# Leo-Liao-Chao/Uncertainty-Aware-CILQR-for-Trajectory-Optimization

Hardware: AMD Instinct MI355X
Metric: CILQR solves/sec (N=50, batch B) (higher is better)
Workload: dtype f64

## Files before the change

### uncertainty-aware-cilqr-for-trajectory-optimization_amd/csrc/cilqr_solve.hip

```cpp
#include <type_traits>

#include "cilqr_device.hpp"

namespace cilqr {

using namespace dev;

namespace {

constexpr int FREC = 16;

__device__ __forceinline__ double readfirstlane_f64(double v) {
  int lo = __double2loint(v), hi = __double2hiint(v);
  lo = __builtin_amdgcn_readfirstlane(lo);
  hi = __builtin_amdgcn_readfirstlane(hi);
  return __hiloint2double(hi, lo);
}

__device__ __forceinline__ double wave_sum(double v) {
#pragma unroll
  for (int o = 32; o > 0; o >>= 1) v += __shfl_xor(v, o, WAVE);
  return v;
}

// ... 358 lines not shown
    riccati_step<!GENERAL>(rb, V, dt, two_wvel, lamb, g, ok);
    if (GENERAL) { if (!ok) return false; } else suspect |= __builtin_amdgcn_ballot_w64(!ok);
    store_gains<RW>(kK, j - 1, g);
  }
  if (j == 0) {
    riccati_step<!GENERAL>(ra, V, dt, two_wvel, lamb, g, ok);
    if (GENERAL) { if (!ok) return false; } else suspect |= __builtin_amdgcn_ballot_w64(!ok);
    store_gains<RW>(kK, 0, g);
  }
  return suspect == 0;
}

#define CILQR_MFMA(xa, xb, xc) __builtin_amdgcn_mfma_f64_4x4x4f64(xa, xb, xc, 0, 0, 0)

__device__ __forceinline__ double readlane_f64(double v, int l) {
  int lo = __double2loint(v), hi = __double2hiint(v);
  lo = __builtin_amdgcn_readlane(lo, l);
  hi = __builtin_amdgcn_readlane(hi, l);
  return __hiloint2double(hi, lo);
}
__device__ __forceinline__ double odd_blocks_from_even(double v) {
  int lo = __double2loint(v), hi = __double2hiint(v);
  lo = __builtin_amdgcn_update_dpp(lo, lo, 0x114, 0xF, 0xA, false);
  hi = __builtin_amdgcn_update_dpp(hi, hi, 0x114, 0xF, 0xA, false);
  return __hiloint2double(hi, lo);
}

struct MfmaOperands { double AB, AA, BB, Ca, Cb; };
struct MfmaCursor {
  const double *AB, *AA, *BB, *Ca, *Cb;
  int sAB, sAA, sBB, sCa, sCb;
  __device__ __forceinline__ void upper(MfmaOperands& o) const { o.AB = AB[RECF]; o.AA = AA[RECF]; o.BB = BB[RECF]; o.Ca = Ca[RECF]; o.Cb = Cb[RECF]; }
  __device__ __forceinline__ void lower(MfmaOperands& o) const { o.AB = AB[0]; o.AA = AA[0]; o.BB = BB[0]; o.Ca = Ca[0]; o.Cb = Cb[0]; }
  __device__ __forceinline__ void back() { AB -= sAB; AA -= sAA; BB -= sBB; Ca -= sCa; Cb -= sCb; }
};

__device__ __forceinline__ void mfma_place(const double*& ptr, int& stride, int slot, const double* low, const double* cst) {
  ptr = slot >= 0 ? low + slot : cst + (-1 - slot);
  stride = slot >= 0 ? 2 * RECF : 0;
}

template <bool FSMEM, bool DIAG>
__device__ __forceinline__ bool riccati_mfma(int N, const double* rec, double* kK, double* fwd, const double* cst, double inv_half_dt, double lamb_in,
                                             unsigned long long* sub) {
  constexpr int C0 = -1, C1 = -2, CDT = -3, CW = -4, C2 = -5;
  const int lane = threadIdx.x;
  const int e = ((lane >> 4) << 2) | (lane & 3);
  const bool odd = (lane & 4) != 0;
  const int slotA = e == 0 || e == 5 || e == 10 || e == 15 ? C1 : e == 2 ? 10 : e == 6 ? 11 : e == 3 ? 12 : e == 7 ? 13 : C0;
  const int slotB = e == 0 ? 10 : e == 4 ? 11 : e == 8 ? C2 : e == 13 ? CDT : C0;
  const int slotXX = e == 0 ? 3 : e == 1 || e == 4 ? 4 : e == 5 ? 5 : e == 10 ? CW : C0;
  const int slotX = e == 2 ? 0 : e == 6 ? 1 : e == 10 ? 2 : C0;
  const int slotUU = e == 0 ? 8 : e == 5 ? 9 : e == 2 ? 6 : e == 6 ? 7 : C0;
  const double* low = rec + (N - 2) * RECF;
  MfmaCursor cur;
  mfma_place(cur.AB, cur.sAB, odd ? slotB : slotA, low, cst);
  mfma_place(cur.AA, cur.sAA, slotA, low, cst);
  mfma_place(cur.BB, cur.sBB, slotB, low, cst);
  mfma_place(cur.Ca, cur.sCa, odd ? slotX : slotXX, low, cst);
  mfma_place(cur.Cb, cur.sCb, odd ? slotUU : C0, low, cst);
  double m00 = e == 0 ? 1.0 : 0.0, m01 = e == 1 || e == 4 ? 1.0 : 0.0, m11 = e == 5 ? 1.0 : 0.0;
  double mvc = odd && (lane & 3) == 2 ? 1.0 : 0.0;
  double lamb = lamb_in, lamb0 = lamb_in * (inv_half_dt * inv_half_dt);
  double lamb_row = (lane >> 4) == 0 ? lamb0 : lamb;
  CILQR_PIN(m00); CILQR_PIN(m01); CILQR_PIN(m11); CILQR_PIN(mvc); CILQR_PIN(lamb); CILQR_PIN(lamb0); CILQR_PIN(lamb_row);
  const bool stores = lane == 6 || lane == 22 || lane < 4 || (lane >= 16 && lane < 20);
  const int gslot = lane == 6 ? 0 : lane == 22 ? 1 : lane < 4 ? 2 + lane : 6 + (lane & 3);
  unsigned goff = stores ? (unsigned)(((N - 1) * FREC + gslot) * 8) : (unsigned)((N * FREC + (lane & 15)) * 8);
  const unsigned gstride = stores ? FREC * 8 : 0;
  char* const gbase = reinterpret_cast<char*>(fwd);
  double* gp = kK + (N - 1) * RECF + (stores ? gslot : 10 + (lane & 3));

  MfmaOperands oa, ob;
  cur.upper(oa);
  double V = odd_blocks_from_even(oa.Ca), vc = oa.Ca * mvc;
  int signs_v = 0, signs_s = 0;
  double det0 = 0.0;
  auto step = [&](const MfmaOperands& o) {
    unsigned long long s0 = 0, s1 = 0, s2 = 0, s3 = 0;
    if (DIAG) stamp_request(s0, V);
    const double P = CILQR_MFMA(V, o.AB, vc);
    const double Db = CILQR_MFMA(o.BB, P, o.Cb);
    const double Da = CILQR_MFMA(o.AA, P, o.Ca);
    const double a = readlane_f64(Db, 4), b = readlane_f64(Db, 5), d = readlane_f64(Db, 21);
    if (DIAG) stamp_request(s1, a + b + d);
    const double bb = b * b;
    det0 = fma(a, d, -bb);
    signs_v |= __double2hiint(det0);
    signs_s |= __double2hiint(a) | __double2hiint(d);
    const double ar = a + lamb0, dr = d + lamb;
    const double nr = -rcp_newton(fma(ar, dr, -bb));
    if (DIAG) stamp_request(s2, nr);
    const double adj = fma(ar, m11, fma(-b, m01, dr * m00));
    const double Dk = CILQR_MFMA(adj, Db, 0.0) * nr;
    const double H0 = fma(lamb_row, Dk, Db);
    const double H = odd_blocks_from_even(H0);
    double Dv = CILQR_MFMA(H, Dk, Da);
    vc = Dv * mvc;
    CILQR_PIN(vc);
    CILQR_PIN(Dv);
    V = odd_blocks_from_even(Dv);
    if (FSMEM) {
      *reinterpret_cast<double*>(gbase + goff) = Dk;
      goff -= gstride;
      asm volatile("" : "+v"(goff));
    } else {
      *gp = Dk;
      gp -= RECF;
    }
    if (DIAG) {
      stamp_request(s3, V);
      stamps_collect(s0, s1, s2, s3);
      sub[5] += s1 - s0; sub[6] += s2 - s1; sub[7] += s3 - s2;
    }
  };
  auto trip = [&] {
    cur.lower(ob);
    step(oa);
    cur.back();
    cur.upper(oa);
    step(ob);
  };
  bool two_left;
  if (FSMEM) {
    two_left = ((N - 1) & 1) != 0;
    for (int trips = (N - 1) >> 1; trips > 0; --trips) trip();
  } else {
    int j = N - 1;
    for (; j >= 2; j -= 2) trip();
    two_left = j == 1;
  }
  if (two_left) {
    cur.lower(ob);
    step(oa);
    step(ob);
  } else {
    step(oa);
  }
  return __builtin_amdgcn_ballot_w64((signs_v | signs_s) < 0 || !(det0 == det0)) == 0;
}

typedef __attribute__((address_space(3))) double lds_f64;
struct MfmaLdsCursor {
  const lds_f64 *AB, *AA, *BB, *Ca, *Cb;
  int sAB, sAA, sBB, sCa, sCb;
  __device__ __forceinline__ void upper(MfmaOperands& o) const { o.AB = AB[RECF]; o.AA = AA[RECF]; o.BB = BB[RECF]; o.Ca = Ca[RECF]; o.Cb = Cb[RECF]; }
  __device__ __forceinline__ void lower(MfmaOperands& o) const { o.AB = AB[0]; o.AA = AA[0]; o.BB = BB[0]; o.Ca = Ca[0]; o.Cb = Cb[0]; }
};
__device__ __forceinline__ void mfma_place(const lds_f64*& ptr, int& stride, int slot, const lds_f64* low, const lds_f64* cst) {
  ptr = slot >= 0 ? low + slot : cst + (-1 - slot);
  stride = slot >= 0 ? 2 * RECF : 0;
}

template <bool DIAG>
__device__ __forceinline__ bool riccati_mfma_smem(int N, const double* rec, double* fwd, const double* cst, double inv_half_dt, double lamb_in,
                                                  unsigned long long* sub) {
  constexpr int C0 = -1, C1 = -2, CDT = -3, CW = -4, C2 = -5;
  const int lane = threadIdx.x;
  const int e = ((lane >> 4) << 2) | (lane & 3);
  const bool odd = (lane & 4) != 0;
  const int slotA = e == 0 || e == 5 || e == 10 || e == 15 ? C1 : e == 2 ? 10 : e == 6 ? 11 : e == 3 ? 12 : e == 7 ? 13 : C0;
  const int slotB = e == 0 ? 10 : e == 4 ? 11 : e == 8 ? C2 : e == 13 ? CDT : C0;
  const int slotXX = e == 0 ? 3 : e == 1 || e == 4 ? 4 : e == 5 ? 5 : e == 10 ? CW : C0;
  const int slotX = e == 2 ? 0 : e == 6 ? 1 : e == 10 ? 2 : C0;
  const int slotUU = e == 0 ? 8 : e == 5 ? 9 : e == 2 ? 6 : e == 6 ? 7 : C0;
  using PTR = const lds_f64*;
  const PTR low = (PTR)rec + (N - 2) * RECF;
  const PTR cstp = (PTR)cst;
  MfmaLdsCursor cur;
  mfma_place(cur.AB, cur.sAB, odd ? slotB : slotA, low, cstp);
  mfma_place(cur.AA, cur.sAA, slotA, low, cstp);
  mfma_place(cur.BB, cur.sBB, slotB, low, cstp);
  mfma_place(cur.Ca, cur.sCa, odd ? slotX : slotXX, low, cstp);
  mfma_place(cur.Cb, cur.sCb, odd ? slotUU : C0, low, cstp);
  double m00 = e == 0 ? 1.0 : 0.0, m01 = e == 1 || e == 4 ? 1.0 : 0.0, m11 = e == 5 ? 1.0 : 0.0;
  double mvc = odd && (lane & 3) == 2 ? 1.0 : 0.0;
  double lamb = lamb_in, lamb0 = lamb_in * (inv_half_dt * inv_half_dt);
  double lamb_row = (lane >> 4) == 0 ? lamb0 : lamb;
  CILQR_PIN(m00); CILQR_PIN(m01); CILQR_PIN(m11); CILQR_PIN(mvc); CILQR_PIN(lamb); CILQR_PIN(lamb0); CILQR_PIN(lamb_row);
  const bool stores = lane == 6 || lane == 22 || lane < 4 || (lane >= 16 && lane < 20);
  const int gslot = lane == 6 ? 0 : lane == 22 ? 1 : lane < 4 ? 2 + lane : 6 + (lane & 3);
  unsigned goff = stores ? (unsigned)(((N - 1) * FREC + gslot) * 8) : (unsigned)((N * FREC + (lane & 15)) * 8);
  const unsigned gstride = stores ? FREC * 8 : 0;
  char* const gbase = reinterpret_cast<char*>(fwd);
  lds_f64* qp = (lds_f64*)rec + (N - 2) * RECF + (lane == 4 ? 0 : lane == 5 ? 1 : lane == 21 ? 2 : 3 + lane % 11);

  MfmaOperands oa, ob;
  cur.upper(oa);
  double V = odd_blocks_from_even(oa.Ca), vc = oa.Ca * mvc;
  auto step = [&](const MfmaOperands& o, auto kind, auto upper_step) {
    constexpr int KIND = decltype(kind)::value, QOFF = decltype(upper_step)::value ? RECF : 0;
    unsigned long long s0 = 0, s1 = 0, s2 = 0, s3 = 0;
    if (DIAG) stamp_request(s0, V);
    const double P = CILQR_MFMA(V, o.AB, vc);
    double Db = CILQR_MFMA(o.BB, P, o.Cb);
    const double Da = CILQR_MFMA(o.AA, P, o.Ca);
    if (KIND != 3) {
      asm volatile("" : "+v"(Db) : "v"(cur.AB), "v"(cur.AA), "v"(cur.BB), "v"(cur.Ca), "v"(cur.Cb));
      if (KIND == 1) cur.upper(oa); else cur.lower(ob);
      asm volatile("");
    }
    const double a = readlane_f64(Db, 4), b = readlane_f64(Db, 5), d = readlane_f64(Db, 21);
    if (DIAG) stamp_request(s1, a + b + d);
    const double bb = b * b;
    const double ar = a + lamb0, dr = d + lamb;
    const double den = fma(ar, dr, -bb);
    const double adj = fma(ar, m11, fma(-b, m01, dr * m00));
    double Dkr = CILQR_MFMA(adj, Db, 0.0);
    double r = __builtin_amdgcn_rcp(den);
    asm volatile("" : "+v"(Dkr), "+v"(r), "+v"(goff) : "v"(qp));
    qp[QOFF] = Db;
    asm volatile("");
    r = fma(fma(-den, r, 1.0), r, r);
    r = fma(fma(-den, r, 1.0), r, r);
    const double nr = -r;
    if (DIAG) stamp_request(s2, nr);
    const double Dk = Dkr * nr;
    double H0 = fma(lamb_row, Dk, Db);
    if (KIND == 0) {
      asm volatile("" : "+v"(H0) : "v"(cur.AB), "v"(cur.AA));
      cur.AB -= cur.sAB; cur.AA -= cur.sAA;
    }
    if (KIND == 1) {
      asm volatile("" : "+v"(H0) : "v"(qp));
      qp -= 2 * RECF;
    }
    double H = odd_blocks_from_even(H0);
    if (KIND == 0) {
      asm volatile("" : "+v"(H) : "v"(cur.BB), "v"(cur.Ca));
      cur.BB -= cur.sBB; cur.Ca -= cur.sCa;
    }
    double Dv = CILQR_MFMA(H, Dk, Da);
    asm volatile("" : "+v"(Dv) : "v"(goff));
    *reinterpret_cast<double*>(gbase + goff) = Dk;
    asm volatile("" : "+v"(Dv) : : "memory");
    vc = Dv * mvc;
    CILQR_PIN(vc);
    asm volatile("" : "+v"(Dv) : "v"(goff), "v"(cur.Cb));
    goff -= gstride;
    if (KIND == 0) cur.Cb -= cur.sCb;
    V = odd_blocks_from_even(Dv);
    if (DIAG) {
      stamp_request(s3, V);
      stamps_collect(s0, s1, s2, s3);
      sub[5] += s1 - s0; sub[6] += s2 - s1; sub[7] += s3 - s2;
    }
  };
  using Upper = std::true_type;
  using Lower = std::false_type;
  using K0 = std::integral_constant<int, 0>;
  using K1 = std::integral_constant<int, 1>;
  using K2 = std::integral_constant<int, 2>;
  using K3 = std::integral_constant<int, 3>;
  for (int trips = (N - 1) >> 1; trips > 0; --trips) {
    step(oa, K0(), Upper());
    step(ob, K1(), Lower());
  }
  if (((N - 1) & 1) != 0) {
    step(oa, K2(), Upper());
    step(ob, K3(), Lower());
  } else {
    step(oa, K3(), Upper());
  }
  bool bad = false;
  for (int base = 0; base < N; base += WAVE) {
    const int t = base + lane;
    const double* q = rec + (t < N ? t : N - 1) * RECF;
    const double a = q[0], b = q[1], d = q[2];
    const double bb = b * b;
    const double det0 = fma(a, d, -bb);
    const int signs = __double2hiint(det0) | __double2hiint(a) | __double2hiint(d);
    bad |= t < N && (signs < 0 || (t == 0 && !(det0 == det0)));
  }
  return __builtin_amdgcn_ballot_w64(bad) == 0;
}

template <int KS>
__device__ __forceinline__ void load_fwd(FwdIn& o, const double* X, const double* U, const double* kK, int i) {
  const double* xo = X + i * XR;
  o.x = xo[0]; o.y = xo[1]; o.v = xo[2]; o.th = xo[3];
  o.u0 = U[2 * i]; o.u1 = U[2 * i + 1];
  const double* g = kK + i * KS;
#pragma unroll
  for (int k = 0; k < KR; ++k) o.g[k] = g[k];
}

__device__ __forceinline__ void fwd_step_store(const FwdConst& k, const FwdIn& c, State& s, double& max_turn, double inv_half_dt,
                                               double* Un_i, double* Xn_next) {
  double u0, u1;
  forward_step<true>(k, c, s, max_turn, u0, u1, inv_half_dt);
  Un_i[0] = u0; Un_i[1] = u1;
  Xn_next[0] = s.x; Xn_next[1] = s.y; Xn_next[2] = s.v; Xn_next[3] = s.th; Xn_next[4] = s.c; Xn_next[5] = s.s;
}

typedef double d2_t __attribute__((ext_vector_type(2)));
typedef __attribute__((address_space(3))) d2_t lds_d2;
constexpr int FSTEP = FREC * 8;
static_assert(XR % 2 == 0, "state records are whole 16-byte pairs");
struct FwdBump {
  unsigned& off;
  lds_d2*& un;
  lds_d2*& xn;
  template <int J> __device__ __forceinline__ void pin(double& ps, double& pc) const {
    if (J == 0) {
      asm volatile("" : "+v"(ps), "+v"(pc) : "v"(un));
      un += 2;
      asm volatile("" : "+v"(un));
    } else if (J == 1) {
      asm volatile("" : "+v"(ps), "+v"(pc) : "v"(xn));
      xn += XR;
      asm volatile("" : "+v"(xn));
    } else if (J == 2) {
      asm volatile("" : "+v"(ps), "+v"(pc) : "s"(off));
      off += 2 * FSTEP;
      asm volatile("" : "+s"(off));
    } else {
      CILQR_PIN2(ps, pc);
    }
  }
};
typedef double d8_t __attribute__((ext_vector_type(8)));
struct FwdS { d8_t lo, hi; };
__device__ __forceinline__ void f_sload_first(FwdS& r, const double* p) {
  asm volatile("s_load_dwordx16 %0, %2, 0x0\n\ts_load_dwordx16 %1, %2, 0x40" : "=&s"(r.lo), "=&s"(r.hi) : "s"(p) : "memory");
}
template <int AHEAD>
__device__ __forceinline__ void f_sload_next(FwdS& r, const double* fwd, unsigned off) {
  asm volatile("s_load_dwordx16 %0, %2, %3 offset:%4\n\ts_load_dwordx16 %1, %2, %3 offset:%5"
               : "+s"(r.lo), "+s"(r.hi) : "s"(fwd), "s"(off), "n"(AHEAD), "n"(AHEAD + 64) : "memory");
}
__device__ __forceinline__ void f_swait(FwdS& r) {
  __builtin_amdgcn_s_waitcnt(0xC07F);
  asm volatile("" : "+s"(r.lo), "+s"(r.hi) : : "memory");
}
__device__ __forceinline__ void f_sunpack(FwdIn& o, const FwdS& r) {
  o.g[0] = r.lo[0]; o.g[1] = r.lo[1]; o.g[2] = r.lo[2]; o.g[3] = r.lo[3]; o.g[4] = r.lo[4]; o.g[5] = r.lo[5];
  o.g[6] = r.lo[6]; o.g[7] = r.lo[7]; o.g[8] = r.hi[0]; o.g[9] = r.hi[1];
  o.x = r.hi[2]; o.y = r.hi[3]; o.v = r.hi[4]; o.th = r.hi[5]; o.u0 = r.hi[6]; o.u1 = r.hi[7];
}

template <bool PUBLISH = false>
__device__ __forceinline__ bool forward_smem(const KParams& kp, int N, const double* X, const double* fwd, double* Xn, double* Un) {
  asm volatile("s_waitcnt vmcnt(0)\n\ts_dcache_inv\n\ts_waitcnt lgkmcnt(0)" ::: "memory");
  FwdConst k;
  make_fwd_const(k, kp);
  double ihd = 2.0 / kp.dt;
  CILQR_PIN(ihd);
  State s;
  s.x = X[0]; s.y = X[1]; s.v = X[2]; s.th = X[3]; s.c = X[4]; s.s = X[5];
  store_state(Xn, 0, s);
  double max_turn = 0.0;
  FwdS r;
  FwdIn c;
  f_sload_first(r, fwd);
  unsigned off = 0;
  lds_d2* un = (lds_d2*)Un;
  lds_d2* xn = (lds_d2*)(Xn + XR);
  asm volatile("" : "+s"(off), "+v"(un), "+v"(xn));
  const FwdBump bump{off, un, xn};
  auto step = [&](auto ahead, auto slot, const auto& pins) {
    constexpr int AHEAD = decltype(ahead)::value, SLOT = decltype(slot)::value;
    f_swait(r);
    f_sunpack(c, r);
    double u0, u1;
    forward_controls_scalar(c, s, u0, u1, ihd);
    f_sload_next<AHEAD>(r, fwd, off);
    un[SLOT] = d2_t{u0, u1};
    const double delta = dyn_pose_loop(k, s, u0, u1, max_turn);
    lds_d2* xo = xn + SLOT * (XR / 2);
    xo[0] = d2_t{s.x, s.y};
    if (PUBLISH) asm volatile("" ::: "memory");
    xo[1] = d2_t{s.v, s.th};
    rotate_heading(k, delta, s.s, s.c, pins);
    CILQR_PIN2(s.s, s.c);
  };
  using I0 = std::integral_constant<int, 0>;
  using I1 = std::integral_constant<int, 1>;
  const unsigned end = (unsigned)N * FSTEP, last = N > 0 ? end - FSTEP : 0;
  while (off < last) {
    step(std::integral_constant<int, FSTEP>(), I0(), PlainPins());
    step(std::integral_constant<int, 2 * FSTEP>(), I1(), bump);
  }
  if (off < end) step(std::integral_constant<int, FSTEP>(), I0(), PlainPins());
  f_swait(r);
  return max_turn <= MAX_TURN;
}

template <int KS>
__device__ __forceinline__ bool forward_fast(const KParams& kp, int N, const double* X, const double* U, const double* kK,
                                             double* Xn, double* Un) {
  FwdConst k;
  make_fwd_const(k, kp);
  double ihd = 2.0 / kp.dt;
  CILQR_PIN(ihd);
  State s;
  s.x = X[0]; s.y = X[1]; s.v = X[2]; s.th = X[3]; s.c = X[4]; s.s = X[5];
  if (threadIdx.x == 0) store_state(Xn, 0, s);
  double max_turn = 0.0;
  FwdIn fa, fb;
  load_fwd<KS>(fa, X, U, kK, 0);
  int i = 0;
  for (; i + 1 < N; i += 2) {
    load_fwd<KS>(fb, X, U, kK, i + 1);
    fwd_step_store(k, fa, s, max_turn, ihd, Un + 2 * i, Xn + (i + 1) * XR);
    load_fwd<KS>(fa, X, U, kK, i + 2 < N ? i + 2 : i + 1);
    fwd_step_store(k, fb, s, max_turn, ihd, Un + 2 * (i + 1), Xn + (i + 2) * XR);
  }
  if (i < N) fwd_step_store(k, fa, s, max_turn, ihd, Un + 2 * i, Xn + (i + 1) * XR);
  return max_turn <= MAX_TURN;
// ... 602 lines not shown
        m = fmax(m, d == d ? d : __builtin_huge_val());
      }
      grid.dmax = wave_max_uniform(m);
    }
    handover = !rollout_fast(kp, N, a.x0 + (size_t)b * 4, Ua, Xa) || (a.flags & CILQR_FLAG_GENERAL_ONLY) != 0;
    if (handover && lane == 0) *reinterpret_cast<volatile int*>(cmd) = CMD_EXIT;
  }
  __syncthreads();

  const int t = lane;
  const bool act = t < N;
  const int n_mine = (M - wave + W - 1) / W;
  if (wave != 0) {
    for (;;) {
      if (*reinterpret_cast<volatile int*>(cmd) == CMD_EXIT) break;
      if (act) {
        const KParams kpl = phase_params();
        const double* xr = Xa + t * XR;
        SampledSource src{tab, off, rmax, Xa, N, NSMP, M, a.samp_w, kpl.ego_front, kpl.ego_rear,
                          sqrt(1.0 + 64.0 / kpl.q2_front), sqrt(1.0 + 64.0 / kpl.q2_rear)};
        src.o_first = wave; src.o_stride = W;
        StepSums s5{0.0, 0.0, 0.0, 0.0, 0.0};
        obstacle_loop<true, false, false, false>(make_obs_consts(kpl, xr[0], xr[1], xr[4], xr[5]), n_mine * NSMP, src.at(t), s5);
        double* q = part + ((size_t)(wave - 1) * N + t) * 5;
        q[0] = s5.lx0; q[1] = s5.lx1; q[2] = s5.h00; q[3] = s5.h01; q[4] = s5.h11;
        if (UNC && wave == W - 1) {
          double g0 = 0.0, g1 = 0.0, h00 = 0.0, h01 = 0.0, h11 = 0.0;
          unc_cost_add(phase_args().unc, upose, b, xr[0], xr[1], xr[4], xr[5], g0, g1, h00, h01, h11);
          double* qu = umap + (size_t)t * 5;
          qu[0] = g0; qu[1] = g1; qu[2] = h00; qu[3] = h01; qu[4] = h11;
        }
      }
      __syncthreads();
      __syncthreads();
    }
    return;
  }

  CILQR_STAMP(c_pro)
  double J_old = DBL_MAX, lamb = 1.0, J_new = 0.0;
  int iters = 0, status = CILQR_EXIT_MAX_ITER, n_pass = 0;
  bool j_valid = false;
  const int max_it = kp.max_iterations;
  for (int it = 0; it < max_it && !handover; ++it) {
    ++iters;
    {
      const KParams kpl = phase_params();
      Rec c{};
      double Jt = 0.0;
      if (act) {
        const double* xr = Xa + t * XR;
        const double* xn = Xa + (t + 1) * XR;
        const int cs = closest_sample<false>(S, grid, xr[0], xr[1], LdsSamples{samp, grid.xf, grid.dxs});
        SampledSource src{tab, off, rmax, Xa, N, NSMP, M, a.samp_w, kpl.ego_front, kpl.ego_rear,
                          sqrt(1.0 + 64.0 / kpl.q2_front), sqrt(1.0 + 64.0 / kpl.q2_rear)};
        src.o_first = 0; src.o_stride = W;
        Jt = lin_step<true, false, false, false>(kpl, xr[0], xr[1], xr[2], xr[4], xr[5], Ua[2 * t], Ua[2 * t + 1], xn[2], xn[4], xn[5],
                                           fma(grid.dxs, (double)cs, grid.xf), samp[cs], n_mine * NSMP, src.at(t), c);
      }
      __syncthreads();
      if (act) {
#pragma unroll
        for (int w = 1; w < W; ++w) {
          const double* q = part + ((size_t)(w - 1) * N + t) * 5;
          c.lx0 += q[0]; c.lx1 += q[1]; c.l00 += q[2]; c.l01 += q[3]; c.l11 += q[4];
        }
        if (UNC) {
          const double* qu = umap + (size_t)t * 5;
          c.lx0 += qu[0]; c.lx1 += qu[1]; c.l00 += qu[2]; c.l01 += qu[3]; c.l11 += qu[4];
        }
        double* r = rec + t * RECF;
        const double ih = 2.0 / kpl.dt;
        r[0] = c.lx0; r[1] = c.lx1; r[2] = c.lx2; r[3] = c.l00; r[4] = c.l01; r[5] = c.l11;
        r[6] = c.lu0 * ih; r[7] = c.lu1; r[8] = c.luu0 * (ih * ih); r[9] = c.luu1;
        r[10] = c.al; r[11] = c.be; r[12] = c.ga; r[13] = c.de;
      }
      J_new = wave_sum_uniform(Jt);
      j_valid = true;
    }
    CILQR_STAMP(c_L)
    if (DIAG) ++n_L;
    const bool accept = J_new < J_old;
    bool stop = false;
    if (!accept) {
      if (J_new != J_new) {
        status = CILQR_EXIT_NUMERIC;
      } else {
        for (;;) {
          lamb = lamb * kp.lamb_factor;
          if (lamb > kp.lamb_max) { status = CILQR_EXIT_LAMBDA_MAX; break; }
          if (++it >= max_it) { status = CILQR_EXIT_MAX_ITER; break; }
          ++iters;
        }
      }
      stop = true;
    } else {
      asm volatile("s_waitcnt lgkmcnt(0)" ::: "memory");
      if (!riccati_mfma<false, false>(N, rec, rec, nullptr, cst, 2.0 / kp.dt, lamb, nullptr)) {
        handover = true;
        stop = true;
      } else {
        CILQR_STAMP(c_R)
        ++n_pass;
        if (DIAG) ++n_R;
        if (!forward_fast<RECF>(KParams(phase_params()), N, Xa, Ua, rec, Xa, Ua)) {
          handover = true;
          stop = true;
        } else {
          j_valid = false;
          lamb = lamb / kp.lamb_factor;
          if (fabs(J_new - J_old) < kp.tolerance) { status = CILQR_EXIT_TOLERANCE; stop = true; }
          J_old = J_new;
          if (it + 1 >= max_it) stop = true;
        }
      }
    }
    if (stop && lane == 0) *reinterpret_cast<volatile int*>(cmd) = CMD_EXIT;
    __syncthreads();
    CILQR_STAMP(c_F)
    if (stop) break;
  }

  int32_t* const hint = phase_args().hint_passes;
  if (lane == 0) {
    phase_args().redo[b] = handover ? 1 : 0;
    if (handover && hint) hint[b] = 63;
  }
  if (handover) return;

  const SolveArgs ae = phase_args();
  double* Uo = ae.U + (size_t)b * 2 * N;
  for (int i = lane; i < 2 * N; i += WAVE) Uo[i] = Ua[i];
  double* Xg = ae.X_out + (size_t)b * 4 * (N + 1);
  for (int i = lane; i < 4 * (N + 1); i += WAVE) Xg[i] = Xa[(i >> 2) * XR + (i & 3)];
  if (ae.J_out) {
    if (!j_valid) J_new = wave_sum_uniform(cost_only(ae.kp, N, lane, samp, S, grid, Xa, Ua));
    if (lane == 0) ae.J_out[b] = J_new;
  }
  if (lane == 0) {
    if (ae.iters_out) ae.iters_out[b] = iters;
    if (ae.status_out) ae.status_out[b] = status;
    if (ae.passes) ae.passes[b] = n_pass;
    if (ae.hint_passes) ae.hint_passes[b] = n_pass;
  }
  if (DIAG && lane == 0 && a.diag) {
    const unsigned long long now_ = __builtin_readcyclecounter();
    unsigned long long* o = a.diag + (size_t)b * DIAG_SLOTS;
    o[0] = c_pro; o[1] = c_L; o[2] = c_R; o[3] = c_F; o[4] = now_ - tk; o[5] = n_L; o[6] = n_R; o[7] = now_ - tk0;
    for (int q = 8; q < DIAG_SLOTS; ++q) o[q] = 0;
  }
#undef CILQR_STAMP
}

template <int W, bool LONG, bool DIAG, bool UNC = false>
__global__ __launch_bounds__(W * WAVE, UNC ? 2 : W) void cilqr_solve_share_kernel(SolveArgs a) {
  static_assert(!(LONG && W != 2), "the long-horizon form is built for two wavefronts");
  constexpr int STEPS = LONG ? 2 : 1;
  unsigned long long tk0 = 0, tk = 0, c_pro = 0, c_L = 0, c_R = 0, c_F = 0, n_L = 0, n_R = 0, c_wait = 0;
  if (DIAG) tk0 = tk = __builtin_readcyclecounter();
#define CILQR_STAMP(acc)                                 \
  if (DIAG) {                                            \
    const unsigned long long now_ = __builtin_readcyclecounter(); \
    acc += now_ - tk;                                    \
    tk = now_;                                           \
  }
  extern __shared__ __attribute__((aligned(16))) double lds[];
  if ((int)blockIdx.x >= a.B) return;
  const int b = __builtin_amdgcn_readfirstlane(a.order ? a.order[blockIdx.x] : (int)blockIdx.x);
  if (b >= a.B) return;
  const int tid = threadIdx.x, lane = tid & (WAVE - 1);
  const int wave = __builtin_amdgcn_readfirstlane(tid >> 6);
  const KParams kp = a.kp;
  const int N = a.N, M = a.M, S = kp.n_samples;
  double* samp = lds;
  double* Xa = samp + ((S + 1) & ~1);
  double* Ua = Xa + (N + 1) * XR;
  double* rec = Ua + 2 * N;
  double* cst = rec + N * RECF;
  double* tab = cst + RCST;
  double* part = tab + (size_t)M * TABF * N;
  double* umap = part + (size_t)(W - 1) * 5 * N;
  double* ctl = part + ((((W - 1) + (UNC ? 1 : 0)) * 5 * N + 1) & ~1);
  int* const cmd = reinterpret_cast<int*>(ctl);
  double* fwd = a.fwd + (size_t)b * (N + 1) * FREC;

  SampleGrid grid;
  make_sample_grid(grid, a.xplan_fl[2 * b], a.xplan_fl[2 * b + 1], S);
  const double* Ug = a.U + (size_t)b * 2 * N;
  for (int i = tid; i < 2 * N; i += W * WAVE) Ua[i] = Ug[i];
  if (tid < 16 && (tid & 7) < 5) cst[(tid & 7) + (tid >> 3) * RECF] = (tid & 7) == 0 ? 0.0 : (tid & 7) == 1 ? 1.0 : (tid & 7) == 2 ? kp.dt : (tid & 7) == 3 ? kp.w_vel * 2 : 2.0;
  if (tid == 0) cmd[0] = 0;
  const double* wts = obs_weights(a, b);
  UncPose upose{0, 0, 1, 0};
  if (UNC) upose = unc_pose(a.unc, b);
  __syncthreads();
  bool handover = false;
  if (wave == 0) {
    handover = !rollout_fast(kp, N, a.x0 + (size_t)b * 4, Ua, Xa) || (a.flags & CILQR_FLAG_GENERAL_ONLY) != 0;
    if (handover && lane == 0) *reinterpret_cast<volatile int*>(cmd) = CMD_EXIT;
  } else {
    const int al = lane + (wave - 1) * WAVE, an = (W - 1) * WAVE;
    for (int i = al; i < M * N; i += an) {
      const int m = i / N;
      const ObsEntry e = obs_entry_at(kp, a, b, m, i - m * N);
      double* o = tab + (size_t)i * TABF;
      o[0] = e.ox; o[1] = e.oy; o[2] = e.co; o[3] = e.so; o[4] = e.ia2; o[5] = e.ib2;
    }
    if (wave == 1) {
      const double* pc = a.poly + (size_t)b * CILQR_POLY_COEFFS;
      for (int s = lane; s < S; s += WAVE) {
        double xs;
        sample_xy(grid, pc, s, xs, samp[s]);
      }
      asm volatile("s_waitcnt lgkmcnt(0)" ::: "memory");
      double m = 0.0;
      for (int q = lane; q + 1 < S; q += WAVE) {
        const double d = fabs(samp[q + 1] - samp[q]);
        m = fmax(m, d == d ? d : __builtin_huge_val());
      }
      m = wave_max_uniform(m);
      const double p2 = path_curvature_wave(grid, pc, S, lane, cst);
      if (lane == 0) { ctl[1] = m; ctl[2] = p2; }
    }
  }
  __syncthreads();
  grid.dmax = ctl[1];
  grid.p2 = ctl[2];
  grid.pc = cst + CST_PC;

  if (wave != 0) {
    unsigned long long busy = 0, calls = 0;
    for (;;) {
      if (*reinterpret_cast<volatile int*>(cmd) == CMD_EXIT) break;
      unsigned long long t0 = 0;
      if (DIAG) t0 = __builtin_readcyclecounter();
      const KParams kpl = phase_params();
      auto aux_step = [&](int t, double cA, double sA, double cn, double sn) {
        const double* xr = Xa + t * XR;
        const double u0 = Ua[2 * t], u1 = Ua[2 * t + 1];
        StepSums s5{0.0, 0.0, 0.0, 0.0, 0.0};
        const ObsConsts oc = make_obs_consts(kpl, xr[0], xr[1], cA, sA);
        if (W == 2 || (UNC && wave == 1)) {
          obstacle_loop<true, false, true>(oc, M, TabSource<false>{tab, wts, N, kpl.w_obstacle}.at(t), s5);
        } else if (!UNC) {
          const int first = wave - 1;
          obstacle_loop<true, false, true, false>(oc, (M - first + 1) / 2, TabObstaclesStrided{tab + (size_t)t * TABF, wts, N, first, 2, kpl.w_obstacle}, s5);
        }
        double* q = part + ((size_t)(wave - 1) * N + t) * 5;
        q[0] = s5.lx0; q[1] = s5.lx1; q[2] = s5.h00; q[3] = s5.h01; q[4] = s5.h11;
        if (UNC && wave == W - 1) {
          double g0 = 0.0, g1 = 0.0, h00 = 0.0, h01 = 0.0, h11 = 0.0;
          unc_cost_add(phase_args().unc, upose, b, xr[0], xr[1], cA, sA, g0, g1, h00, h01, h11);
          double* qu = umap + (size_t)t * 5;
          qu[0] = g0; qu[1] = g1; qu[2] = h00; qu[3] = h01; qu[4] = h11;
        }
        if (wave == W - 1) {
          Rec c;
          ab_terms(kpl, u0, Xa[(t + 1) * XR + 2], cn, sn, c);
          double* r = rec + t * RECF;
          r[10] = c.al; r[11] = c.be; r[12] = c.ga; r[13] = c.de;
        }
        if (W == 3 && wave == (UNC ? 1 : 2)) {
          Rec c;
          double a1, a2, a3, a4;
          ctrl_args(kpl, u0, u1, xr[2], a1, a2, a3, a4);
          const double e1 = exp_fast(a1);
          const double e2 = exp_fast(a2);
          const double e3 = exp_fast(a3);
          const double e4 = exp_fast(a4);
          ctrl_terms(kpl, u0, u1, e1, e2, e3, e4, c);
          double* r = rec + t * RECF;
          const double ih = 2.0 / kpl.dt;
          r[6] = c.lu0 * ih; r[7] = c.lu1; r[8] = c.luu0 * (ih * ih); r[9] = c.luu1;
        }
      };
      double cn = 0.0;
      if (!LONG) {
        double sA = 0.0, cA = 1.0;
        if (lane <= N) sincos_loop(Xa[lane * XR + 3], sA, cA);
        cn = __shfl_down(cA, 1, WAVE);
        double sn = __shfl_down(sA, 1, WAVE);
        if (N == WAVE && lane == WAVE - 1 && wave == W - 1) sincos_loop(Xa[N * XR + 3], sn, cn);
        if (lane < N) aux_step(lane, cA, sA, cn, sn);
      } else {
        for (int t = lane; t < N; t += WAVE) {
          double sA, cA, sn = 0.0;
          sincos_loop(Xa[t * XR + 3], sA, cA);
          cn = 1.0;
          if (wave == W - 1) sincos_loop(Xa[(t + 1) * XR + 3], sn, cn);
          aux_step(t, cA, sA, cn, sn);
        }
      }
      if (DIAG) { busy += stamp_after(cn) - t0; ++calls; }
      __syncthreads();
      __syncthreads();
    }
    if (DIAG && lane == 0 && a.diag && wave == 1) {
      unsigned long long* o = a.diag + (size_t)b * DIAG_SLOTS;
      o[8] = busy; o[9] = calls;
    }
    if (DIAG && lane == 0 && a.diag)
      a.diag[(size_t)b * DIAG_SLOTS + 12 + wave] = (unsigned long long)__builtin_amdgcn_s_getreg((4) | (0 << 6) | (31 << 11)) |
                                                    ((unsigned long long)__builtin_amdgcn_s_getreg((20) | (0 << 6) | (31 << 11)) << 32);
    if (DIAG && lane == 0 && a.diag && wave == 2) a.diag[(size_t)b * DIAG_SLOTS + 11] = busy;
    return;
  }

  CILQR_STAMP(c_pro)
  double J_old = DBL_MAX, lamb = 1.0, J_new = 0.0;
  int iters = 0, status = CILQR_EXIT_MAX_ITER, n_pass = 0;
  bool j_valid = false;
  const int max_it = kp.max_iterations;
  for (int it = 0; it < max_it && !handover; ++it) {
    ++iters;
    {
      const KParams kpl = phase_params();
      double dx[STEPS], dy[STEPS], lx2[STEPS], Jt = 0.0;
#pragma unroll
      for (int c2 = 0; c2 < STEPS; ++c2) {
        dx[c2] = 0.0; dy[c2] = 0.0; lx2[c2] = 0.0;
        const int t = lane + c2 * WAVE;
        if (t < N) {
          const double* xr = Xa + t * XR;
          const double px = xr[0], py = xr[1], v = xr[2];
          const double u0 = Ua[2 * t], u1 = Ua[2 * t + 1];
          double2* q = reinterpret_cast<double2*>(fwd + t * FREC + 10);
          q[0] = make_double2(px, py);
          q[1] = make_double2(v, xr[3]);
          q[2] = make_double2(u0, u1);
          const int cs = closest_sample(S, grid, px, py, LdsSamples{samp, grid.xf, grid.dxs});
          dx[c2] = px - fma(grid.dxs, (double)cs, grid.xf);
          dy[c2] = py - samp[cs];
          const double dv = v - kpl.desired_speed;
          lx2[c2] = (2 * kpl.w_vel) * dv;
          Jt += stage_cost(kpl, dx[c2], dy[c2], dv, u0, u1);
          if (W == 2) {
            Rec c;
            double a1, a2, a3, a4;
            ctrl_args(kpl, u0, u1, v, a1, a2, a3, a4);
            const double e1 = exp_fast(a1);
            const double e2 = exp_fast(a2);
            const double e3 = exp_fast(a3);
            const double e4 = exp_fast(a4);
            ctrl_terms(kpl, u0, u1, e1, e2, e3, e4, c);
            double* r = rec + t * RECF;
            const double ih = 2.0 / kpl.dt;
            r[6] = c.lu0 * ih; r[7] = c.lu1; r[8] = c.luu0 * (ih * ih); r[9] = c.luu1;
          }
        }
      }
      J_new = wave_sum_uniform(Jt);
      unsigned long long w0 = 0;
      if (DIAG) w0 = stamp_after(J_new);
      __syncthreads();
      if (DIAG) c_wait += __builtin_readcyclecounter() - w0;
#pragma unroll
      for (int c2 = 0; c2 < STEPS; ++c2) {
        const int t = lane + c2 * WAVE;
        if (t < N) {
          const double* q = part + (size_t)t * 5;
          StepSums s5{q[0], q[1], q[2], q[3], q[4]};
          if (W == 3 && !UNC) {
            const double* qo = q + (size_t)N * 5;
            s5.lx0 += qo[0]; s5.lx1 += qo[1]; s5.h00 += qo[2]; s5.h01 += qo[3]; s5.h11 += qo[4];
          }
          double* r = rec + t * RECF;
          double lx0, lx1, l00, l01, l11;
          state_terms(kpl, dx[c2], dy[c2], s5, lx0, lx1, l00, l01, l11);
          if (UNC) {
            const double* qu = umap + (size_t)t * 5;
            lx0 += qu[0]; lx1 += qu[1]; l00 += qu[2]; l01 += qu[3]; l11 += qu[4];
          }
          r[0] = lx0; r[1] = lx1; r[2] = lx2[c2]; r[3] = l00; r[4] = l01; r[5] = l11;
        }
      }
      j_valid = true;
    }
    CILQR_STAMP(c_L)
    if (DIAG) ++n_L;
    const bool accept = J_new < J_old;
    bool stop = false;
    if (!accept) {
      if (J_new != J_new) {
        status = CILQR_EXIT_NUMERIC;
      } else {
        for (;;) {
          lamb = lamb * kp.lamb_factor;
          if (lamb > kp.lamb_max) { status = CILQR_EXIT_LAMBDA_MAX; break; }
          if (++it >= max_it) { status = CILQR_EXIT_MAX_ITER; break; }
          ++iters;
        }
      }
      stop = true;
    } else {
      asm volatile("s_waitcnt lgkmcnt(0)" ::: "memory");
      if (!(W == 3 ? riccati_mfma<true, false>(N, rec, rec, fwd, cst, 2.0 / kp.dt, lamb, nullptr)
                   : riccati_mfma_smem<false>(N, rec, fwd, cst, 2.0 / kp.dt, lamb, nullptr))) {
        handover = true;
        stop = true;
      } else {
        CILQR_STAMP(c_R)
        ++n_pass;
        if (DIAG) ++n_R;
        if (!forward_smem(KParams(phase_params()), N, Xa, fwd, Xa, Ua)) {
          handover = true;
          stop = true;
        } else {
          j_valid = false;
          lamb = lamb / kp.lamb_factor;
          if (fabs(J_new - J_old) < kp.tolerance) { status = CILQR_EXIT_TOLERANCE; stop = true; }
          J_old = J_new;
          if (it + 1 >= max_it) stop = true;
        }
      }
    }
    if (stop && lane == 0) *reinterpret_cast<volatile int*>(cmd) = CMD_EXIT;
    __syncthreads();
    CILQR_STAMP(c_F)
    if (stop) break;
  }

  int32_t* const hint = phase_args().hint_passes;
  if (lane == 0) {
    phase_args().redo[b] = handover ? 1 : 0;
    if (handover && hint) hint[b] = 63;
  }
  if (handover) return;

  const SolveArgs ae = phase_args();
  double* Uo = ae.U + (size_t)b * 2 * N;
  for (int i = lane; i < 2 * N; i += WAVE) Uo[i] = Ua[i];
  double* Xg = ae.X_out + (size_t)b * 4 * (N + 1);
  for (int i = lane; i < 4 * (N + 1); i += WAVE) Xg[i] = Xa[(i >> 2) * XR + (i & 3)];
  if (ae.J_out) {
    if (!j_valid) J_new = wave_sum_uniform(cost_only(ae.kp, N, lane, samp, S, grid, Xa, Ua));
    if (lane == 0) ae.J_out[b] = J_new;
  }
  if (lane == 0) {
    if (ae.iters_out) ae.iters_out[b] = iters;
    if (ae.status_out) ae.status_out[b] = status;
    if (ae.passes) ae.passes[b] = n_pass;
    if (ae.hint_passes) ae.hint_passes[b] = n_pass;
  }
  if (DIAG && lane == 0 && a.diag) {
    const unsigned long long now_ = __builtin_readcyclecounter();
    unsigned long long* o = a.diag + (size_t)b * DIAG_SLOTS;
    o[0] = c_pro; o[1] = c_L; o[2] = c_R; o[3] = c_F; o[4] = now_ - tk; o[5] = n_L; o[6] = n_R; o[7] = now_ - tk0;
    o[10] = c_wait;
    o[12] = (unsigned long long)__builtin_amdgcn_s_getreg((4) | (0 << 6) | (31 << 11)) |
            ((unsigned long long)__builtin_amdgcn_s_getreg((20) | (0 << 6) | (31 << 11)) << 32);
    if (W == 2) { o[11] = 0; o[14] = 0; }
    o[15] = 0;
  }
#undef CILQR_STAMP
}

__global__ void quu_inverse_kernel(int n, const double* q, const double* lamb, double* out, int general) {
  const int i = blockIdx.x * blockDim.x + threadIdx.x;
  if (i >= n) return;
  const double a = q[4 * i], b = 0.5 * (q[4 * i + 1] + q[4 * i + 2]), d = q[4 * i + 3];
  double i00 = 0, i01 = 0, i11 = 0;
  bool ok = true;
  if (general) ok = quu_inverse_general(a, b, d, lamb[i], i00, i01, i11);
  else quu_inverse_psd(a, b, d, lamb[i], b * b, i00, i01, i11);
  const double nan = __builtin_nan("");
  out[4 * i] = ok ? i00 : nan; out[4 * i + 1] = ok ? i01 : nan; out[4 * i + 2] = ok ? i01 : nan; out[4 * i + 3] = ok ? i11 : nan;
}

__global__ void closest_sample_kernel(int n, int S, const double* in, int32_t* out) {
  const int i = blockIdx.x * blockDim.x + threadIdx.x;
  if (i >= n) return;
  const double* q = in + (size_t)i * 10;
  double pc[CILQR_POLY_COEFFS];
  for (int j = 0; j < CILQR_POLY_COEFFS; ++j) pc[j] = q[j];
  SampleGrid g;
  make_sample_grid(g, q[6], q[7], S);
  auto at = [&](int s, double& x, double& y) { sample_xy(g, pc, s, x, y); };
  double m = 0.0, A = 0.0, B = 0.0, yp = 0.0;
  for (int s = 0; s < S; ++s) {
    double x, y, a2, a3;
    at(s, x, y);
    if (s > 0) { const double d = fabs(y - yp); m = fmax(m, d == d ? d : __builtin_huge_val()); }
    yp = y;
    path_curvature_terms(pc, x, a2, a3);
    A = fmax(A, a2 == a2 ? a2 : __builtin_huge_val());
    B = fmax(B, a3 == a3 ? a3 : __builtin_huge_val());
  }
  g.dmax = m;
  g.p2 = path_curvature_bound(g, pc, S, A, B);
  g.pc = pc;
  const double px = q[8], py = q[9];
  XWindow w = closest_window_x(S, g, px, py, at);
  closest_window_y(S, g, px, py, w);
  const int by_newton = w.hi - w.lo >= NEWTON_MIN_WINDOW ? closest_newton(S, g, px, py, at, w) : -1;
  out[3 * (size_t)i] = closest_sample(S, g, px, py, at);
  out[3 * (size_t)i + 1] = closest_scan(0, S - 1, px, py, at);
  out[3 * (size_t)i + 2] = by_newton >= 0 ? 1 : 0;
}

__global__ void unc_cost_kernel(UncArgs u, int n, const double* states, double* cost, double* vx, double* mx) {
  const int i = blockIdx.x * blockDim.x + threadIdx.x;
  if (i >= n) return;
  const UncPose po = unc_pose(u, 0);
  const double* st = states + 4 * (size_t)i;
  double sn, cs;
  sincos_fast(st[3], &sn, &cs);
  double g0 = 0.0, g1 = 0.0, h00 = 0.0, h01 = 0.0, h11 = 0.0;
  const double c = unc_cost_add(u, po, 0, st[0], st[1], cs, sn, g0, g1, h00, h01, h11);
  const double inv = u.scale != 0.0 ? 1.0 / (u.scale * (double)(u.nl * u.nw)) : 0.0;
  cost[i] = c;
  vx[2 * i] = g0 * inv; vx[2 * i + 1] = g1 * inv;
  mx[3 * i] = h00 * inv; mx[3 * i + 1] = h01 * inv; mx[3 * i + 2] = h11 * inv;
}

template <typename F>
hipError_t with_bool(bool b, F&& f) {
  return b ? f(std::true_type{}) : f(std::false_type{});
}
template <typename F>
hipError_t with_bools(bool b1, bool b2, F&& f) {
  return with_bool(b1, [&](auto c1) { return with_bool(b2, [&](auto c2) { return f(c1, c2); }); });
}

}

__global__ __launch_bounds__(1024) void schedule_order_kernel(const int32_t* passes, int B, int32_t* order) {
  __shared__ int cnt[64], base[64];
  const int tid = threadIdx.x;
  if (tid < 64) cnt[tid] = 0;
  __syncthreads();
  for (int i = tid; i < B; i += 1024) {
    const int p = passes[i];
    atomicAdd(&cnt[63 - (p < 0 ? 0 : p > 63 ? 63 : p)], 1);
  }
  __syncthreads();
  if (tid == 0) {
    int acc = 0;
    for (int k = 0; k < 64; ++k) { base[k] = acc; acc += cnt[k]; }
  }
  __syncthreads();
  for (int i = tid; i < B; i += 1024) {
    const int p = passes[i];
    order[atomicAdd(&base[63 - (p < 0 ? 0 : p > 63 ? 63 : p)], 1)] = i;
  }
}

hipError_t launch_schedule_order(const int32_t* passes, int B, int32_t* order, hipStream_t stream) {
  if (B <= 0) return hipSuccess;
  hipLaunchKernelGGL(schedule_order_kernel, dim3(1), dim3(1024), 0, stream, passes, B, order);
  return hipGetLastError();
}

hipError_t launch_unc_cost(const UncArgs& u, int n, const double* states, double* cost, double* vx, double* mx, hipStream_t stream) {
  if (n <= 0) return hipSuccess;
  hipLaunchKernelGGL(unc_cost_kernel, dim3((n + 63) / 64), dim3(64), 0, stream, u, n, states, cost, vx, mx);
  return hipGetLastError();
}

hipError_t launch_closest_sample(int n, int S, const double* in, int32_t* out, hipStream_t stream) {
  if (n <= 0) return hipSuccess;
  hipLaunchKernelGGL(closest_sample_kernel, dim3((n + 63) / 64), dim3(64), 0, stream, n, S, in, out);
  return hipGetLastError();
}

hipError_t launch_quu_inverse(int n, const double* q, const double* lamb, double* out, int general, hipStream_t stream) {
  if (n <= 0) return hipSuccess;
  hipLaunchKernelGGL(quu_inverse_kernel, dim3((n + 63) / 64), dim3(64), 0, stream, n, q, lamb, out, general);
  return hipGetLastError();
}

hipError_t launch_solve_wave(const SolveArgs& a, const WavePlan& p, hipStream_t stream) {
  if (a.B <= 0) return hipSuccess;
  if (p.too_large) return hipErrorInvalidValue;
  if (p.shared_table)
    if (const hipError_t e = launch_obstacle_table(a, stream)) return e;
  using Kernel = void (*)(SolveArgs);
  const auto go = [&](Kernel fast, Kernel general) {
    const size_t want = p.lds_fast > p.lds_general ? p.lds_fast : p.lds_general;
    hipError_t e = hipSuccess;
    for (Kernel k : {fast, general})
      if (want > SOLVE_LDS_DEFAULT && e == hipSuccess) e = hipFuncSetAttribute(reinterpret_cast<const void*>(k), hipFuncAttributeMaxDynamicSharedMemorySize, (int)want);
    void* args[] = {const_cast<SolveArgs*>(&a)};
    if (e == hipSuccess) e = hipLaunchKernel(reinterpret_cast<const void*>(fast), dim3(a.B), dim3(p.W * WAVE), args, p.lds_fast, stream);
    if (e == hipSuccess) e = hipLaunchKernel(reinterpret_cast<const void*>(general), dim3(a.B), dim3(WAVE), args, p.lds_general, stream);
    return e;
  };
  const bool diag = a.diag != nullptr, unc = a.unc.layer != nullptr;
  if (p.kernel == WavePlan::SPLIT)
    return with_bools(diag, unc, [&](auto d, auto u) {
      return p.W == 4 ? go(cilqr_solve_split_kernel<4, d.value, u.value>, cilqr_solve_kernel<d.value, 2, true, u.value>)
                      : go(cilqr_solve_split_kernel<2, d.value, u.value>, cilqr_solve_kernel<d.value, 2, true, u.value>);
    });
  if (p.tab == 2)
    return with_bools(diag, unc, [&](auto d, auto u) { return go(cilqr_solve_kernel<d.value, 2, false, u.value>, cilqr_solve_kernel<d.value, 2, true, u.value>); });
  if (p.kernel == WavePlan::PAIR)
    return with_bool(diag, [&](auto d) { return go(cilqr_solve_pair_kernel<d.value>, cilqr_solve_kernel<d.value, 1, true, false>); });
  if (p.kernel == WavePlan::SHARE)
    return with_bools(unc, diag, [&](auto u, auto d) {
      if (p.long_form) return go(cilqr_solve_share_kernel<2, true, d.value, u.value>, cilqr_solve_kernel<d.value, 1, true, u.value>);
      return p.W == 3 ? go(cilqr_solve_share_kernel<3, false, d.value, u.value>, cilqr_solve_kernel<d.value, 1, true, u.value>)
                      : go(cilqr_solve_share_kernel<2, false, d.value, u.value>, cilqr_solve_kernel<d.value, 1, true, u.value>);
    });
  return with_bool(diag, [&](auto d) {
    return p.tab == 1 ? with_bool(unc, [&](auto u) { return go(cilqr_solve_kernel<d.value, 1, false, u.value>, cilqr_solve_kernel<d.value, 1, true, u.value>); })
                      : with_bool(unc, [&](auto u) { return go(cilqr_solve_kernel<d.value, 0, false, u.value>, cilqr_solve_kernel<d.value, 0, true, u.value>); });
// ... 5 lines not shown
```

Before: 2.556 million.

## Split aux-wave obstacle terms into two rounds overlapping the backward Riccati sweep

In the two-wave share kernel, the helper wave now computes obstacle cost terms in two rounds: first the later half of the horizon, then the earlier half. The backward Riccati pass needs the later stages first, so the main wave can start it after the first round and wait at an LDS barrier partway through. The helper wave finishes the early-stage terms and writes them into the record buffer while the main wave is still in the sweep. The intent is to hide the helper wave's obstacle work behind the Riccati recurrence. In exchange the code adds extra barriers, two lanes per stage with DPP reductions, and more complex barrier matching between the waves.

```diff
diff --git a/uncertainty-aware-cilqr-for-trajectory-optimization_amd/csrc/cilqr_solve.hip b/uncertainty-aware-cilqr-for-trajectory-optimization_amd/csrc/cilqr_solve.hip
--- a/uncertainty-aware-cilqr-for-trajectory-optimization_amd/csrc/cilqr_solve.hip
+++ b/uncertainty-aware-cilqr-for-trajectory-optimization_amd/csrc/cilqr_solve.hip
@@ -534,9 +534,11 @@
   stride = slot >= 0 ? 2 * RECF : 0;
 }
 
-template <bool DIAG>
+__device__ __forceinline__ void lds_barrier() { asm volatile("s_waitcnt lgkmcnt(0)\n\ts_barrier" ::: "memory"); }
+
+template <bool DIAG, int SEG = 0>
 __device__ __forceinline__ bool riccati_mfma_smem(int N, const double* rec, double* fwd, const double* cst, double inv_half_dt, double lamb_in,
-                                                  unsigned long long* sub) {
+                                                  unsigned long long* sub, int seg_trips = 0, unsigned long long* seg_wait = nullptr) {
   constexpr int C0 = -1, C1 = -2, CDT = -3, CW = -4, C2 = -5;
   const int lane = threadIdx.x;
   const int e = ((lane >> 4) << 2) | (lane & 3);
@@ -634,9 +636,24 @@
   using K1 = std::integral_constant<int, 1>;
   using K2 = std::integral_constant<int, 2>;
   using K3 = std::integral_constant<int, 3>;
-  for (int trips = (N - 1) >> 1; trips > 0; --trips) {
-    step(oa, K0(), Upper());
-    step(ob, K1(), Lower());
+  if (SEG) {
+    for (int trips = seg_trips; trips > 0; --trips) {
+      step(oa, K0(), Upper());
+      step(ob, K1(), Lower());
+    }
+    unsigned long long w0 = 0;
+    if (SEG == 2) w0 = stamp_after(V);
+    lds_barrier();
+    if (SEG == 2) *seg_wait += __builtin_readcyclecounter() - w0;
+    for (int trips = ((N - 1) >> 1) - seg_trips; trips > 0; --trips) {
+      step(oa, K0(), Upper());
+      step(ob, K1(), Lower());
+    }
+  } else {
+    for (int trips = (N - 1) >> 1; trips > 0; --trips) {
+      step(oa, K0(), Upper());
+      step(ob, K1(), Lower());
+    }
   }
   if (((N - 1) & 1) != 0) {
     step(oa, K2(), Upper());
@@ -1545,11 +1562,16 @@
 #undef CILQR_STAMP
 }
 
+constexpr int SHARE_SPLIT_MIN = 24;
+__device__ __forceinline__ int share_split(int N) { return N >= SHARE_SPLIT_MIN ? N >> 1 : 0; }
+__device__ __forceinline__ int share_seg_trips(int N) { return N >= SHARE_SPLIT_MIN ? (N - 1 - (N >> 1)) >> 1 : 0; }
+
 template <int W, bool LONG, bool DIAG, bool UNC = false>
 __global__ __launch_bounds__(W * WAVE, UNC ? 2 : W) void cilqr_solve_share_kernel(SolveArgs a) {
   static_assert(!(LONG && W != 2), "the long-horizon form is built for two wavefronts");
   constexpr int STEPS = LONG ? 2 : 1;
-  unsigned long long tk0 = 0, tk = 0, c_pro = 0, c_L = 0, c_R = 0, c_F = 0, n_L = 0, n_R = 0, c_wait = 0;
+  constexpr bool TWO_ROUNDS = W == 2 && !LONG && !UNC;
+  unsigned long long tk0 = 0, tk = 0, c_pro = 0, c_L = 0, c_R = 0, c_F = 0, n_L = 0, n_R = 0, c_wait = 0, c_wait2 = 0;
   if (DIAG) tk0 = tk = __builtin_readcyclecounter();
 #define CILQR_STAMP(acc)                                 \
   if (DIAG) {                                            \
@@ -1622,7 +1644,7 @@
   grid.pc = cst + CST_PC;
 
   if (wave != 0) {
-    unsigned long long busy = 0, calls = 0;
+    unsigned long long busy = 0, calls = 0, busy1 = 0, busy2 = 0;
     for (;;) {
       if (*reinterpret_cast<volatile int*>(cmd) == CMD_EXIT) break;
       unsigned long long t0 = 0;
@@ -1668,6 +1690,51 @@
         }
       };
       double cn = 0.0;
+      if (TWO_ROUNDS) {
+        auto round = [&](int t0, int cnt, bool finish) {
+          const int t = t0 + (lane >> 1), chain = lane & 1;
+          const bool on = lane < 2 * cnt;
+          double so = 0.0, co = 1.0;
+          if (on) sincos_loop(Xa[(t + chain) * XR + 3], so, co);
+          const double cA = dpp_f64<0xA0>(co), sA = dpp_f64<0xA0>(so);
+          StepSums s5{0.0, 0.0, 0.0, 0.0, 0.0};
+          if (on) {
+            const double* xr = Xa + t * XR;
+            obstacle_loop<true, false, true, false>(make_obs_consts(kpl, xr[0], xr[1], cA, sA), (M - chain + 1) / 2,
+                                                    TabObstaclesStrided{tab + (size_t)t * TABF, wts, N, chain, 2, kpl.w_obstacle}, s5);
+            if (chain) {
+              Rec c;
+              ab_terms(kpl, Ua[2 * t], Xa[(t + 1) * XR + 2], co, so, c);
+              double* r = rec + t * RECF;
+              r[10] = c.al; r[11] = c.be; r[12] = c.ga; r[13] = c.de;
+            }
+          }
+          const StepSums odd{dpp_f64<0xF5>(s5.lx0), dpp_f64<0xF5>(s5.lx1), dpp_f64<0xF5>(s5.h00), dpp_f64<0xF5>(s5.h01), dpp_f64<0xF5>(s5.h11)};
+          if (on && !chain) {
+            s5.lx0 += odd.lx0; s5.lx1 += odd.lx1; s5.h00 += odd.h00; s5.h01 += odd.h01; s5.h11 += odd.h11;
+            if (!finish) {
+              double* q = part + (size_t)t * 5;
+              q[0] = s5.lx0; q[1] = s5.lx1; q[2] = s5.h00; q[3] = s5.h01; q[4] = s5.h11;
+            } else {
+              double* r = rec + t * RECF;
+              double lx0, lx1, l00, l01, l11;
+              state_terms(kpl, r[0], r[1], s5, lx0, lx1, l00, l01, l11);
+              r[0] = lx0; r[1] = lx1; r[3] = l00; r[4] = l01; r[5] = l11;
+            }
+          }
+          cn = co;
+        };
+        const int h = share_split(N);
+        round(h, N - h, false);
+        if (DIAG) busy1 += stamp_after(cn) - t0;
+        __syncthreads();
+        if (DIAG) t0 = __builtin_readcyclecounter();
+        if (h > 0) round(0, h, true);
+        if (DIAG) { busy2 += stamp_after(cn) - t0; ++calls; }
+        __syncthreads();
+        __syncthreads();
+        continue;
+      }
       if (!LONG) {
         double sA = 0.0, cA = 1.0;
         if (lane <= N) sincos_loop(Xa[lane * XR + 3], sA, cA);
@@ -1690,7 +1757,8 @@
     }
     if (DIAG && lane == 0 && a.diag && wave == 1) {
       unsigned long long* o = a.diag + (size_t)b * DIAG_SLOTS;
-      o[8] = busy; o[9] = calls;
+      o[8] = TWO_ROUNDS ? busy1 + busy2 : busy; o[9] = calls;
+      if (TWO_ROUNDS) { o[11] = busy1; o[14] = busy2; }
     }
     if (DIAG && lane == 0 && a.diag)
       a.diag[(size_t)b * DIAG_SLOTS + 12 + wave] = (unsigned long long)__builtin_amdgcn_s_getreg((4) | (0 << 6) | (31 << 11)) |
@@ -1708,6 +1776,7 @@
     ++iters;
     {
       const KParams kpl = phase_params();
+      const int split = TWO_ROUNDS ? __builtin_amdgcn_readfirstlane(share_split(phase_args().N)) : 0;
       double dx[STEPS], dy[STEPS], lx2[STEPS], Jt = 0.0;
 #pragma unroll
       for (int c2 = 0; c2 < STEPS; ++c2) {
@@ -1727,6 +1796,10 @@
           const double dv = v - kpl.desired_speed;
           lx2[c2] = (2 * kpl.w_vel) * dv;
           Jt += stage_cost(kpl, dx[c2], dy[c2], dv, u0, u1);
+          if (TWO_ROUNDS && t < split) {
+            double* r = rec + t * RECF;
+            r[0] = dx[c2]; r[1] = dy[c2]; r[2] = lx2[c2];
+          }
           if (W == 2) {
             Rec c;
             double a1, a2, a3, a4;
@@ -1750,7 +1823,7 @@
 #pragma unroll
       for (int c2 = 0; c2 < STEPS; ++c2) {
         const int t = lane + c2 * WAVE;
-        if (t < N) {
+        if (t < N && (!TWO_ROUNDS || t >= split)) {
           const double* q = part + (size_t)t * 5;
           StepSums s5{q[0], q[1], q[2], q[3], q[4]};
           if (W == 3 && !UNC) {
@@ -1785,9 +1858,11 @@
         }
       }
       stop = true;
+      if (TWO_ROUNDS) lds_barrier();
     } else {
       asm volatile("s_waitcnt lgkmcnt(0)" ::: "memory");
       if (!(W == 3 ? riccati_mfma<true, false>(N, rec, rec, fwd, cst, 2.0 / kp.dt, lamb, nullptr)
+            : TWO_ROUNDS ? riccati_mfma_smem<false, DIAG ? 2 : 1>(N, rec, fwd, cst, 2.0 / kp.dt, lamb, nullptr, __builtin_amdgcn_readfirstlane(share_seg_trips(phase_args().N)), &c_wait2)
                    : riccati_mfma_smem<false>(N, rec, fwd, cst, 2.0 / kp.dt, lamb, nullptr))) {
         handover = true;
         stop = true;
@@ -1842,8 +1917,8 @@
     o[10] = c_wait;
     o[12] = (unsigned long long)__builtin_amdgcn_s_getreg((4) | (0 << 6) | (31 << 11)) |
             ((unsigned long long)__builtin_amdgcn_s_getreg((20) | (0 << 6) | (31 << 11)) << 32);
-    if (W == 2) { o[11] = 0; o[14] = 0; }
-    o[15] = 0;
+    if (W == 2 && !TWO_ROUNDS) { o[11] = 0; o[14] = 0; }
+    o[15] = TWO_ROUNDS ? c_wait2 : 0;
   }
 #undef CILQR_STAMP
 }
```

After: 2.597 million (median of 6 runs). 1.6% higher.
